# luigiba/OpenKEonSpark

Measured on AMD Instinct MI355X. Metric: positive triples/sec (training step), higher is better.
Workload: dtype f32

## Files before the change

### openkeonspark_amd/csrc/abi.hip

```cpp
#include <cstdio>
#include <cstring>
#include <iostream>

#include "engine.hpp"

namespace kge {

Engine &engine() {
    static Engine e;
    return e;
}

void set_error(const std::string &msg) {
    engine().last_error = msg;
    std::fprintf(stderr, "[kge_mi355] error: %s\n", msg.c_str());
}

int fail(int code, const std::string &msg) {
    set_error(msg);
    return code;
}

int hip_check(hipError_t e, const char *what) {
    if (e == hipSuccess) return KGE_OK;
// ... 17 lines not shown
    size_t bytes = sizeof(T) * (count ? count : 1);
    int rc = hip_check(hipMalloc(&dst, bytes), what);
    if (rc) return rc;
    if (count) rc = hip_check(hipMemcpy(dst, src, sizeof(T) * count, hipMemcpyHostToDevice), what);
    return rc;
}

int ensure_device_index() {
    Engine &e = engine();
    if (!e.index.loaded) return fail(KGE_ERR_NO_DATASET, "no training set imported (importTrainFiles / kge_import_train_arrays)");
    if (!device_ok()) return fail(KGE_ERR_NO_DEVICE, "no usable HIP device: the sampler has no CPU fallback");
    int rc = KGE_OK;
    if (!e.dev.uploaded) {
        const KgIndex &ix = e.index;
        if ((rc = upload(e.dev.pos, ix.pos.data(), ix.pos.size(), "upload pos"))) return rc;
        if ((rc = upload(e.dev.grp, ix.grp.data(), ix.grp.size(), "upload grp"))) return rc;
        if ((rc = upload(e.dev.ht, ix.ht.data(), ix.ht.size(), "upload ht"))) return rc;
        if ((rc = upload(e.dev.tails_hr, ix.tails_hr.data(), ix.tails_hr.size(), "upload tails"))) return rc;
        if ((rc = upload(e.dev.heads_tr, ix.heads_tr.data(), ix.heads_tr.size(), "upload heads"))) return rc;
        if ((rc = upload(e.dev.rels_ht, ix.rels_ht.data(), ix.rels_ht.size(), "upload rels"))) return rc;
        if ((rc = upload(e.dev.bern_prob, ix.bern_prob.data(), ix.bern_prob.size(), "upload bern"))) return rc;
        e.dev.uploaded = true;
    }
    if ((int64_t)e.streams.size() != e.work_threads) {
        e.streams.assign((size_t)e.work_threads, 0);
        e.dev.streams_sync = 0;
    }
    if (e.dev.streams_sync == 0) {
        if (e.dev.streams_cap < e.work_threads) {
            uint64_t *base = e.dev.streams < e.dev.streams_next ? e.dev.streams : e.dev.streams_next;
            if (base) (void)hipFree(base);
            e.dev.streams = e.dev.streams_next = nullptr;
            if ((rc = hip_check(hipMalloc(&e.dev.streams, sizeof(uint64_t) * 2 * (size_t)e.work_threads), "alloc streams"))) return rc;
            e.dev.streams_next = e.dev.streams + e.work_threads;
            e.dev.streams_cap = e.work_threads;
        }
        if ((rc = hip_check(hipMemcpy(e.dev.streams, e.streams.data(), sizeof(uint64_t) * (size_t)e.work_threads,
                                      hipMemcpyHostToDevice), "upload streams"))) return rc;
        e.dev.streams_sync = 1;
    }
    return KGE_OK;
}

int ensure_typed_host_index() {
    Engine &e = engine();
    if (!e.index.loaded) return fail(KGE_ERR_NO_DATASET, "type-constrained sampling: no training set imported");
// ... 31 lines not shown
    if (e.dev.streams_sync == 2) {
        int rc = hip_check(hipMemcpy(e.streams.data(), e.dev.streams, sizeof(uint64_t) * e.streams.size(),
                                     hipMemcpyDeviceToHost), "download streams");
        if (rc) return rc;
        e.dev.streams_sync = 1;
    }
    return KGE_OK;
}

static void adopt_index(KgIndex &&ix) {
    Engine &e = engine();
    e.index = std::move(ix);
    e.dev.uploaded = false;
}

static std::string build_and_adopt(int64_t E, int64_t R, int64_t nb, int64_t n, const int64_t *h, const int64_t *t, const int64_t *r) {
    Engine &e = engine();
    if (device_ok()) { (void)flush_attached_sampler(nullptr); (void)hipDeviceSynchronize(); }
    if (e.index_device_min >= 0 && n >= e.index_device_min && device_ok() && device_index_build_supported(E, R, n)) {
        KgIndex ix;
        std::string err = build_index_device(ix, e.dev, E, R, nb, n, h, t, r);
        if (!err.empty()) { e.dev.uploaded = false; return err; }
        e.index = std::move(ix);
        return "";
    }
    KgIndex ix;
    std::string err = build_index(ix, E, R, nb, n, h, t, r);
    if (!err.empty()) return err;
    adopt_index(std::move(ix));
    return "";
}

void transe_team_shape(int D, int &L, int &C);
}

using namespace kge;

extern "C" {

void setInPath(char *path) {
    engine().in_path = path ? path : "";
    std::printf("Input Files Path : %s\n", engine().in_path.c_str());
}

void setOutPath(char *path) {
    engine().out_path = path ? path : "";
    std::printf("Output Files Path : %s\n", engine().out_path.c_str());
}

void setWorkThreads(INT threads) { engine().work_threads = threads < 1 ? 1 : threads; }
INT getWorkThreads(void) { return engine().work_threads; }
void setBern(INT con) { engine().bern = con; }
// ... 55 lines not shown
    if (hip_check(hipMemcpy(batch_h, w, sizeof(int64_t) * total, hipMemcpyDeviceToHost), "copy batch_h")) return;
    if (hip_check(hipMemcpy(batch_t, w + total, sizeof(int64_t) * total, hipMemcpyDeviceToHost), "copy batch_t")) return;
    if (hip_check(hipMemcpy(batch_r, w + 2 * total, sizeof(int64_t) * total, hipMemcpyDeviceToHost), "copy batch_r")) return;
    hip_check(hipMemcpy(batch_y, w + 3 * total, sizeof(float) * total, hipMemcpyDeviceToHost), "copy batch_y");
}

size_t kge_last_error(char *buf, size_t n) {
    const std::string &s = engine().last_error;
    if (buf && n) {
        size_t k = s.size() < n - 1 ? s.size() : n - 1;
        std::memcpy(buf, s.data(), k);
        buf[k] = 0;
    }
    return s.size();
}

void kge_clear_error(void) { engine().last_error.clear(); }
int kge_device_available(void) { return device_ok() ? 1 : 0; }
const char *kge_version(void) { return "kge_mi355 0.1 (gfx950)"; }

int kge_set_option(const char *name, INT value) {
    std::string n = name ? name : "";
    if (n == "counts_force_sort") { engine().counts_force_sort = value != 0; return KGE_OK; }
    if (n == "ride_shares") { engine().ride_shares = (int)value; return KGE_OK; }
    if (n == "transr_bf16x3") { engine().transr_bf16x3 = value != 0; return KGE_OK; }
    if (n == "transr_groups") { engine().transr_groups = (int)value; return KGE_OK; }
    if (n == "transr_fuse_vec") { engine().transr_fuse_vec = value != 0; return KGE_OK; }
    if (n == "counts_fused") { engine().counts_fused = value != 0; return KGE_OK; }
    if (n == "counts_fused_diag") { engine().counts_fused_diag = (int)value; return KGE_OK; }
    if (n == "counts_fused_cap") { engine().counts_fused_cap = value > 0 ? (int)value : 0; return KGE_OK; }
    if (n == "inv_table_max_bytes") { engine().inv_table_max_bytes = value; return KGE_OK; }
    if (n == "tables_changed") { tables_written(); return KGE_OK; }
    if (n == "counts_krel") { int k = 1; while (k * 2 <= value && k < 64) k *= 2; engine().counts_krel = k; return KGE_OK; }
    if (n == "inv_carry") { engine().inv_carry = value != 0; tables_written(); return KGE_OK; }
    if (n == "emit_rounds") { engine().emit_rounds = value != 0; return KGE_OK; }
    if (n == "emit_pack") { engine().emit_pack = value != 0; return KGE_OK; }
    if (n == "float_records") { engine().float_records = value != 0; return KGE_OK; }
    if (n == "float_records_min") { engine().float_records_min = value; return KGE_OK; }
    if (n == "index_device_min") { engine().index_device_min = value; return KGE_OK; }
    if (n == "hub_copies") { engine().hub_copies = value != 0; return KGE_OK; }
    if (n == "pair_counts") { engine().pair_counts = value != 0; return KGE_OK; }
    if (n == "record_emit_event") { engine().record_emit_event = value != 0; return KGE_OK; }
    if (n == "transr_dgrad_records") { engine().transr_dgrad_records = value != 0; return KGE_OK; }
    if (n == "transr_dgrad_records_min") { engine().transr_dgrad_records_min = value; return KGE_OK; }
    if (n == "transr_lean") { engine().transr_lean = value != 0; return KGE_OK; }
    if (n == "pair_counts_min_neg") { engine().pair_counts_min_neg = (int)value; return KGE_OK; }
// ... 51 lines not shown
int kge_import_train_arrays(INT ent_total, INT rel_total, INT n, const INT *h, const INT *t, const INT *r,
                            INT new_batch_total) {
    std::string err = build_and_adopt(ent_total, rel_total, new_batch_total, n, (const int64_t *)h, (const int64_t *)t,
                                      (const int64_t *)r);
    if (!err.empty()) return fail(KGE_ERR_BAD_ARG, err);
    return KGE_OK;
}

int64_t kge_index_copy(const char *what, void *dst, int64_t bytes) {
    const KgIndex &ix = engine().index;
    if (!ix.loaded) return fail(KGE_ERR_NO_DATASET, "kge_index_copy: no dataset");
    const void *src = nullptr;
    int64_t have = 0;
    std::string w = what ? what : "";
    const bool typed = w == "type_tails" || w == "type_heads" || w == "type_bounds" || w == "typed_pos_hr" || w == "typed_pos_tr" ||
                       w == "typed_len";
    if (typed) { int rc = ensure_typed_host_index(); if (rc) return rc; }
#define KGE_ARR(name, vec) if (w == name) { src = (vec).data(); have = (int64_t)((vec).size() * sizeof((vec)[0])); }
    KGE_ARR("tails_hr", ix.tails_hr) KGE_ARR("heads_tr", ix.heads_tr) KGE_ARR("rels_ht", ix.rels_ht)
    KGE_ARR("pos", ix.pos) KGE_ARR("grp", ix.grp) KGE_ARR("ht", ix.ht)
    KGE_ARR("left_mean", ix.left_mean) KGE_ARR("right_mean", ix.right_mean) KGE_ARR("bern_prob", ix.bern_prob)
    KGE_ARR("type_tails", ix.type_tails) KGE_ARR("type_heads", ix.type_heads) KGE_ARR("type_bounds", ix.type_bounds)
    KGE_ARR("typed_pos_hr", ix.typed_pos_hr) KGE_ARR("typed_pos_tr", ix.typed_pos_tr) KGE_ARR("typed_len", ix.typed_len)
#undef KGE_ARR
    if (!src && have == 0 && !typed && w != "tails_hr" && w != "heads_tr" && w != "rels_ht" && w != "pos" && w != "grp" && w != "ht" &&
        w != "left_mean" && w != "right_mean" && w != "bern_prob")
        return fail(KGE_ERR_BAD_ARG, "kge_index_copy: unknown array " + w);
    if (dst && bytes > 0 && have > 0) std::memcpy(dst, src, (size_t)(bytes < have ? bytes : have));
    return have;
}

int kge_set_typed_sampling(INT on) {
    Engine &e = engine();
    int rc = flush_attached_sampler(nullptr);
    if (rc) return rc;
    if (on && (rc = ensure_typed_host_index())) return rc;
    e.typed_sampling = on ? 1 : 0;
    return KGE_OK;
}

int kge_typed_sampling(void) { return engine().typed_sampling; }

int kge_get_stream_states(uint64_t *dst, INT n) {
    Engine &e = engine();
    int rc = pull_streams();
    if (rc) return rc;
    for (INT i = 0; i < n && i < (INT)e.streams.size(); i++) dst[i] = e.streams[(size_t)i];
    return KGE_OK;
// ... 205 lines not shown
```

### openkeonspark_amd/csrc/engine.hpp

```cpp
#pragma once
#include <hip/hip_runtime.h>

#include <cstdint>
#include <mutex>
#include <string>
#include <vector>

#include "../../include/kge_mi355.h"
#include "kg_index.hpp"

namespace kge {

struct DeviceIndex {
    bool uploaded = false;
    int4 *pos = nullptr;
    int4 *grp = nullptr;
    int2 *ht = nullptr;
    int32_t *tails_hr = nullptr, *heads_tr = nullptr, *rels_ht = nullptr;
    float *bern_prob = nullptr;
    uint64_t *streams = nullptr;
    uint64_t *streams_next = nullptr;
    int64_t streams_cap = 0;
    int streams_sync = 0;
    int32_t *stage_i32 = nullptr;
    int64_t *stage_i64 = nullptr;
    int64_t stage_cap = 0;
    float *loss_partials = nullptr;
    unsigned *loss_ticket = nullptr;
    bool typed_uploaded = false;
    int2 *typed_len = nullptr;
    int4 *type_bounds = nullptr;
    int32_t *type_tails = nullptr, *type_heads = nullptr, *typed_pos_hr = nullptr, *typed_pos_tr = nullptr;
};

struct Engine {
    std::mutex mu;
    std::string in_path = "../data/FB15K/";
    std::string out_path = "../data/FB15K/";
    int64_t work_threads = 1;
    int64_t bern = 0;
    KgIndex index;
    LibcRand libc;
    std::vector<uint64_t> streams;
    LcgJumpTable jump = make_jump_table();
    DeviceIndex dev;
    std::string last_error;
    int device_state = 0;
    int record_emit_event = 0;
    hipEvent_t emit_done = nullptr;
    unsigned long long emit_seq = 0, emit_waited = 0;
    int time_emit = 0;
    static constexpr int kEmitRing = 512;
    hipEvent_t ev_emit0[kEmitRing] = {}, ev_emit1[kEmitRing] = {};
    long long emit_launches = 0;
    long long emit_seen = 0;
    int time_sampler = 0;
    hipEvent_t ev_samp0[kEmitRing] = {}, ev_samp1[kEmitRing] = {};
    long long samp_launches = 0, samp_seen = 0;
    float *inv_norm = nullptr;
    int64_t inv_cap = 0;
    const float *inv_for_ent = nullptr, *inv_for_rel = nullptr;
    int inv_valid = 0;
    int32_t *loss_limbs = nullptr;
    int counts_krel = 4;
    int inv_carry = 1;
    int emit_rounds = 1;
    int emit_pack = 1;
// ... 124 lines not shown
```

### openkeonspark_amd/csrc/kg_index.cpp

```cpp
#include "kg_index.hpp"

#include <algorithm>
#include <cstdio>
#include <cstdlib>
#include <cstring>
#include <numeric>

namespace kge {

namespace {

bool slurp(const std::string &path, std::vector<char> &buf) {
    FILE *f = std::fopen(path.c_str(), "rb");
    if (!f) return false;
    std::fseek(f, 0, SEEK_END);
    long n = std::ftell(f);
    std::fseek(f, 0, SEEK_SET);
    buf.resize(static_cast<size_t>(n) + 1);
    size_t got = n > 0 ? std::fread(buf.data(), 1, static_cast<size_t>(n), f) : 0;
    buf[got] = 0;
    buf.resize(got + 1);
    std::fclose(f);
    return true;
}
// ... 236 lines not shown
    f_ = (f_ + 1) % 31;
    r_ = (r_ + 1) % 31;
    return int32_t(v >> 1);
}

LcgJumpTable make_jump_table() {
    LcgJumpTable tab;
    uint64_t a = kLcgMul, c = kLcgAdd;
    for (int j = 0; j < 64; j++) {
        tab.mulA[j] = a;
        tab.addC[j] = c;
        c = a * c + c;
        a = a * a;
    }
    return tab;
}

uint64_t lcg_jump(const LcgJumpTable &tab, uint64_t state, uint64_t steps) {
    for (int j = 0; steps; j++, steps >>= 1)
        if (steps & 1) state = tab.mulA[j] * state + tab.addC[j];
    return state;
}

}
```

### openkeonspark_amd/csrc/kg_index.hpp

```cpp
#pragma once
#include <cstdint>
#include <string>
#include <vector>

namespace kge {

struct Int4 { int32_t x, y, z, w; };
struct Int2 { int32_t x, y; };

struct KgIndex {
    int64_t ent_total = 0, rel_total = 0;
    int64_t train_dup = 0;
    int64_t train_uniq = 0;
    int64_t new_batch = 0;
    std::vector<Int4> pos;
    std::vector<Int4> grp;
    std::vector<Int2> ht;
    std::vector<int32_t> tails_hr;
    std::vector<int32_t> heads_tr;
    std::vector<int32_t> rels_ht;
    std::vector<float> left_mean, right_mean, bern_prob;
    bool loaded = false;
    std::vector<int32_t> type_tails, type_heads;
    std::vector<Int4> type_bounds;
    std::vector<int32_t> typed_pos_hr, typed_pos_tr;
    std::vector<Int2> typed_len;
    bool typed_built = false;
};

std::string load_openke_dir(const std::string &dir, int64_t &ent_total, int64_t &rel_total, int64_t &new_batch,
                            std::vector<int64_t> &h, std::vector<int64_t> &t, std::vector<int64_t> &r);

bool read_all_longs(const std::string &path, std::vector<int64_t> &out);

std::string build_index(KgIndex &ix, int64_t ent_total, int64_t rel_total, int64_t new_batch, int64_t n,
                        const int64_t *h, const int64_t *t, const int64_t *r);

void relation_means(KgIndex &ix, const std::vector<int64_t> &freq_rel, const std::vector<int64_t> &groups_hr,
                    const std::vector<int64_t> &groups_tr);

std::string build_typed_index(KgIndex &ix, const std::vector<int32_t> &head_lef, const std::vector<int32_t> &head_rig,
                              const std::vector<int32_t> &head_type, const std::vector<int32_t> &tail_lef,
                              const std::vector<int32_t> &tail_rig, const std::vector<int32_t> &tail_type);

class LibcRand {
   public:
    LibcRand();
    int32_t next();

   private:
    uint32_t s_[31];
    int f_, r_;
};

constexpr uint64_t kLcgMul = 25214903917ULL;
constexpr uint64_t kLcgAdd = 11ULL;
struct LcgJumpTable { uint64_t mulA[64]; uint64_t addC[64]; };
LcgJumpTable make_jump_table();
uint64_t lcg_jump(const LcgJumpTable &tab, uint64_t state, uint64_t steps);

inline void thread_slice(int64_t batch, int64_t threads, int64_t id, int64_t &lef, int64_t &rig) {
    if (batch % threads == 0) {
        lef = id * (batch / threads);
        rig = (id + 1) * (batch / threads);
    } else {
        lef = id * (batch / threads + 1);
        rig = (id + 1) * (batch / threads + 1);
        if (rig > batch) rig = batch;
        if (lef > batch) lef = batch;
    }
}

}
```

### openkeonspark_amd/csrc/persist.hip

```cpp
#include "models_dev.hpp"
#include "optim_dev.hpp"
#include "sampler_dev.hpp"
#include "team_shape.hpp"

namespace kge {
namespace {

constexpr int kLine = 32;
constexpr unsigned kSpinLimit = 1u << 22;

struct GridBarrier {
    unsigned xcd_count[8 * kLine];
    unsigned xcd_gen[8 * kLine];
    unsigned xcd_pop[8 * kLine];
    unsigned top_count[kLine];
    unsigned flat[kLine];
    unsigned abort_flag[kLine];
};

__device__ __forceinline__ unsigned ld_agent(const unsigned *p) { return __hip_atomic_load(p, __ATOMIC_RELAXED, __HIP_MEMORY_SCOPE_AGENT); }

struct BarrierState {
    unsigned xcc, pop, n_xcd, gen;
};
// ... 330 lines not shown
                if (g_hub_auxr) (void)hipFree(g_hub_auxr);
                g_hub_rel = g_hub_auxr = nullptr;
                g_hub_elems = copies * per_copy;
                if ((rc = hip_check(hipMalloc(&g_hub_rel, sizeof(float) * (size_t)g_hub_elems), "alloc hub copies"))) return rc;
                if ((rc = hip_check(hipMalloc(&g_hub_auxr, sizeof(float) * (size_t)g_hub_elems), "alloc hub copies"))) return rc;
                if ((rc = hip_check(hipMemset(g_hub_rel, 0, sizeof(float) * (size_t)g_hub_elems), "zero hub copies"))) return rc;
                if ((rc = hip_check(hipMemset(g_hub_auxr, 0, sizeof(float) * (size_t)g_hub_elems), "zero hub copies"))) return rc;
            }
            a.copies_rel = g_hub_rel; a.copies_auxr = g_hub_auxr; a.hub_k = (int)copies;
            pa.fold_k = (int)copies; pa.fold_elems = per_copy;
        }
    }
    SamplerArgs &s = pa.sm;
    s.pos = e.dev.pos; s.grp = e.dev.grp; s.ht = e.dev.ht;
    s.tails_hr = e.dev.tails_hr; s.heads_tr = e.dev.heads_tr; s.rels_ht = e.dev.rels_ht;
    s.bern_prob = e.dev.bern_prob; s.streams = e.dev.streams; s.streams_next = nullptr; s.W = W; s.B = B;
    s.out_h = g_batch; s.out_t = g_batch + batch_len; s.out_r = g_batch + 2 * batch_len;
    s.per_thread = (B % W == 0) ? B / W : B / W + 1; s.pos_lo = 0; s.n_local = B; s.out_stride = B;
    s.train_dup = e.index.train_dup; s.new_batch = e.index.new_batch;
    s.ent_total = (int)e.index.ent_total; s.rel_total = (int)e.index.rel_total;
    s.neg = (int)negRate; s.negrel = (int)negRelRate; s.bern = e.bern ? 1 : 0;
    s.pick_div = (unsigned long long)(s.new_batch > 0 ? s.new_batch : s.train_dup);
    s.pick_magic = ~0ull / s.pick_div;
    int kshift = 0;
    while ((1 << kshift) < 1 + negRate + negRelRate) kshift++;
    s.kshift = kshift;
    for (int i = 0; i < 4; i++) { pa.tb.p[i] = pa.tb.g[i] = pa.tb.m[i] = pa.tb.v[i] = nullptr; pa.tb.n[i] = 0; }
    for (int i = 0; i < n_tables; i++) {
        int64_t rows = 0, cols = 0;
        if (kge_table_shape(m, i, &rows, &cols)) return KGE_ERR_BAD_ARG;
        pa.tb.p[i] = tables[i]; pa.tb.g[i] = grads[i]; pa.tb.n[i] = rows * cols;
        if (adam) { pa.tb.m[i] = adam_m[i]; pa.tb.v[i] = adam_v[i]; }
        uintptr_t bits = reinterpret_cast<uintptr_t>(tables[i]) | reinterpret_cast<uintptr_t>(grads[i]);
        if (adam) bits |= reinterpret_cast<uintptr_t>(adam_m[i]) | reinterpret_cast<uintptr_t>(adam_v[i]);
        if (!tables[i] || !grads[i] || (bits & 15)) return fail(KGE_ERR_BAD_ARG, "kge_train_steps_persistent: tables must be non-null and 16-byte aligned");
    }
    pa.n_tables = n_tables; pa.adam = adam; pa.n_steps = (int)n_steps;
    pa.b1 = beta1; pa.b2 = beta2; pa.eps = eps;
    pa.lr = g_lr; pa.losses = d_losses; pa.partials = g_partials; pa.bar = g_bar;
    pa.B = B; pa.W = (int)W;
    pa.touch = e.persist_touch; pa.ahead = e.persist_ahead;
    if (e.persist_trace) {
        if (!g_trace && (rc = hip_check(hipMalloc(&g_trace, sizeof(unsigned long long) * (6 * kTraceSteps + kTraceBlocks)), "alloc phase trace"))) return rc;
        if ((rc = hip_check(hipMemsetAsync(g_trace, 0, sizeof(unsigned long long) * (6 * kTraceSteps + kTraceBlocks), stream), "zero phase trace"))) return rc;
        pa.trace = g_trace;
    }
// ... 50 lines not shown
```

### openkeonspark_amd/csrc/sampler.hip

```cpp
#include "sampler_dev.hpp"

namespace kge {

__global__ __launch_bounds__(256) void sample_kernel_wide(SamplerArgs a) { sample_block_wide(a, blockIdx.x, gridDim.x); }

__global__ __launch_bounds__(256) void sample_kernel(SamplerArgs a) {
    __shared__ float bern_lds[kBernLds];
    sample_block(a, blockIdx.x, gridDim.x, bern_lds);
}

__global__ __launch_bounds__(256) void sample_kernel_wide_typed(TypedSamplerArgs a) { sample_block_wide<true>(a, blockIdx.x, gridDim.x); }

__global__ __launch_bounds__(256) void sample_kernel_typed(TypedSamplerArgs a) {
    __shared__ float bern_lds[kBernLds];
    sample_block<true>(a, blockIdx.x, gridDim.x, bern_lds);
}

__global__ __launch_bounds__(256) void sample_kernel_part(SamplerArgs a) {
    __shared__ float bern_lds[kBernLds];
    sample_block_ride(a, blockIdx.x, bern_lds);
}

__global__ void advance_streams_kernel(uint64_t *streams, long long W, long long B, long long per_thread,
                                       unsigned long long draws) {
// ... 24 lines not shown
    const int64_t W = e.work_threads;
    if (B <= 0 || neg < 0 || negrel < 0 || thread_lo < 0 || thread_hi > W || thread_lo > thread_hi)
        return fail(KGE_ERR_BAD_ARG, "kge_sampling_device: bad batch/thread range");
    if (e.index.train_dup <= 0) return fail(KGE_ERR_NO_DATASET, "sampling: empty training set");
    if ((rc = upload_jump_table())) return rc;
    int64_t lo, hi, tmp;
    if (thread_lo == thread_hi) { lo = hi = 0; }
    else { thread_slice(B, W, thread_lo, lo, tmp); thread_slice(B, W, thread_hi - 1, tmp, hi); }
    const int64_t n_local = hi - lo;
    if (n_local_out) *n_local_out = n_local;
    if (out_stride < n_local) return fail(KGE_ERR_BAD_ARG, "kge_sampling_device: out_stride smaller than the slice");
    const int64_t per_thread = (B % W == 0) ? B / W : B / W + 1;
    a = TypedSamplerArgs();
    a.pos = e.dev.pos; a.grp = e.dev.grp; a.ht = e.dev.ht;
    a.tails_hr = e.dev.tails_hr; a.heads_tr = e.dev.heads_tr; a.rels_ht = e.dev.rels_ht;
    a.bern_prob = e.dev.bern_prob; a.streams = e.dev.streams;
    a.out_h = d_h; a.out_t = d_t; a.out_r = d_r;
    a.per_thread = per_thread; a.pos_lo = lo; a.n_local = n_local; a.out_stride = out_stride;
    a.train_dup = e.index.train_dup; a.new_batch = e.index.new_batch;
    a.ent_total = (int)e.index.ent_total; a.rel_total = (int)e.index.rel_total;
    a.neg = (int)neg; a.negrel = (int)negrel; a.bern = e.bern ? 1 : 0;
    a.pick_div = (unsigned long long)(a.new_batch > 0 ? a.new_batch : a.train_dup);
    a.pick_magic = ~0ull / a.pick_div;
    const int kshift = sampler_kshift(neg, negrel);
    a.kshift = kshift;
    a.pack = emit_pack_shape(a.ent_total, a.rel_total, neg, negrel) ? d_pack : nullptr;
    a.streams_next = e.dev.streams_next; a.W = W; a.B = B;
    if (e.typed_sampling) {
        a.typed_len = e.dev.typed_len; a.type_bounds = e.dev.type_bounds;
        a.type_tails = e.dev.type_tails; a.type_heads = e.dev.type_heads;
        a.typed_pos_hr = e.dev.typed_pos_hr; a.typed_pos_tr = e.dev.typed_pos_tr;
    }
    wide = kshift > 6;
    int64_t nb = n_local > 0 ? ((n_local << kshift) + 255) / 256 : 0;
    if (nb > (1 << 20)) nb = 1 << 20;
    blocks = (unsigned)nb;
    return KGE_OK;
}

static void launch_whole(const TypedSamplerArgs &a, unsigned blocks, bool wide, hipStream_t stream) {
    Engine &e = engine();
    const int slot = (int)(e.samp_launches % Engine::kEmitRing);
    const bool timed = e.time_sampler > 0 && (e.samp_seen++ % e.time_sampler) == 0;
    if (timed) {
        if (!e.ev_samp0[slot]) { (void)hipEventCreate(&e.ev_samp0[slot]); (void)hipEventCreate(&e.ev_samp1[slot]); }
        (void)hipEventRecord(e.ev_samp0[slot], stream);
// ... 89 lines not shown
```

### openkeonspark_amd/csrc/sampler_dev.hpp

```cpp
#pragma once
#include "engine.hpp"

namespace kge {

static __constant__ LcgJumpTable c_jump;
static bool g_jump_uploaded = false;

static inline int upload_jump_table() {
    if (g_jump_uploaded) return KGE_OK;
    int rc = hip_check(hipMemcpyToSymbol(HIP_SYMBOL(c_jump), &engine().jump, sizeof(LcgJumpTable)), "upload jump table");
    if (rc == KGE_OK) g_jump_uploaded = true;
    return rc;
}

struct SamplerArgs {
    const int4 *pos;
    const int4 *grp;
    const int2 *ht;
    const int32_t *tails_hr, *heads_tr, *rels_ht;
    const float *bern_prob;
    const uint64_t *streams;
    uint64_t *streams_next;
    long long W, B;
    int32_t *out_h, *out_t, *out_r;
    int32_t *pack;
    long long per_thread;
    long long pos_lo;
    long long n_local;
    long long out_stride;
    long long train_dup, new_batch;
    unsigned long long pick_div, pick_magic;
    int ent_total, rel_total;
    int neg, negrel, bern;
    int kshift;
    unsigned ride_first, ride_total;
};

struct TypedSamplerArgs : SamplerArgs {
    const int2 *typed_len = nullptr;
    const int4 *type_bounds = nullptr;
    const int32_t *type_tails = nullptr, *type_heads = nullptr, *typed_pos_hr = nullptr, *typed_pos_tr = nullptr;
};
template <bool TYPED> struct SamplerArgsOf { using type = SamplerArgs; };
template <> struct SamplerArgsOf<true> { using type = TypedSamplerArgs; };

__device__ __forceinline__ uint64_t lcg_step(uint64_t s) { return s * kLcgMul + kLcgAdd; }

__device__ __forceinline__ uint64_t lcg_skip(uint64_t s, uint64_t n) {
    for (int j = 0; n != 0; ++j, n >>= 1)
        if (n & 1) s = c_jump.mulA[j] * s + c_jump.addC[j];
    return s;
}

__device__ __forceinline__ uint64_t mod_magic(uint64_t s, uint64_t d, uint64_t m) {
    uint64_t r = s - __umul64hi(s, m) * d;
    while (r >= d) r -= d;
    return r;
}
__device__ __forceinline__ uint32_t mod_u64_u32(uint64_t s, uint32_t d) {
    if (d == 0) return 0;
    const double rcp = 1.0 / (double)d;
    const uint32_t hi = (uint32_t)(s >> 32), lo = (uint32_t)s;
    uint32_t q1 = (uint32_t)((double)hi * rcp);
    int64_t r1 = (int64_t)hi - (int64_t)q1 * d;
    if (r1 < 0) r1 += d;
    if (r1 >= (int64_t)d) r1 -= d;
    const uint64_t x = ((uint64_t)r1 << 32) | lo;
    const double xd = (double)(uint32_t)r1 * 4294967296.0 + (double)lo;
    uint64_t q2 = (uint64_t)(xd * rcp);
    int64_t r2 = (int64_t)(x - q2 * d);
    if (r2 < 0) r2 += d;
    if (r2 < 0) r2 += d;
    if (r2 >= (int64_t)d) r2 -= d;
    if (r2 >= (int64_t)d) r2 -= d;
    return (uint32_t)r2;
}

__device__ __forceinline__ int filtered_pick(const int32_t *__restrict__ vals, int len, long long tmp) {
    int lo = 0, hi = len;
    while (lo < hi) {
        int mid = (lo + hi) >> 1;
        if ((long long)vals[mid] - mid <= tmp) lo = mid + 1; else hi = mid;
    }
    return (int)(tmp + lo);
}

__device__ __forceinline__ int filtered_pick_short(const int32_t *__restrict__ vals, int len, long long tmp) {
    if (len > 4) return filtered_pick(vals, len, tmp);
    if (len <= 0) return (int)tmp;
    int v[4];
#pragma unroll
    for (int j = 0; j < 4; j++) v[j] = vals[j < len ? j : len - 1];
    int lo = 0;
#pragma unroll
    for (int j = 0; j < 4; j++) lo += (j < len && (long long)v[j] - j <= tmp) ? 1 : 0;
    return (int)(tmp + lo);
}

template <bool SHORT>
__device__ __forceinline__ int typed_pick(const TypedSamplerArgs &a, uint64_t s, bool new_tail, int r, const int4 &gq, const int2 &tl) {
    const int32_t *__restrict__ vals = new_tail ? a.typed_pos_hr + gq.x : a.typed_pos_tr + gq.z;
    const int len = new_tail ? tl.x : tl.y;
    int v[4] = {0, 0, 0, 0};
    if (SHORT) {
        const int last = len > 0 ? len - 1 : 0;
#pragma unroll
        for (int j = 0; j < 4; j++) v[j] = vals[j < last ? j : last];
    }
    const int4 tb = a.type_bounds[r];
    const int loff = new_tail ? tb.x : tb.z, llen = new_tail ? tb.y : tb.w;
    const int c = llen - len;
    if (c <= 0) return -1;
    const long long tmp = (long long)mod_u64_u32(s, (uint32_t)c);
    int pos;
    if (SHORT && len <= 4) {
        int lo = 0;
#pragma unroll
        for (int j = 0; j < 4; j++) lo += (j < len && (long long)v[j] - j <= tmp) ? 1 : 0;
        pos = (int)(tmp + lo);
    } else
        pos = filtered_pick(vals, len, tmp);
    pos = min(pos, llen - 1);
    return (new_tail ? a.type_tails : a.type_heads)[loff + pos];
}

__device__ __forceinline__ uint64_t lcg_skip_lanes(uint64_t s, unsigned n) {
#pragma unroll
    for (int j = 0; j < 16; j++) {
        if (!__any((n >> j) != 0u)) break;
        const uint64_t t = c_jump.mulA[j] * s + c_jump.addC[j];
        s = ((n >> j) & 1u) ? t : s;
    }
    return s;
}

template <bool TYPED = false>
__device__ __forceinline__ void sample_slot(const typename SamplerArgsOf<TYPED>::type &a, long long p, long long k, unsigned long long skip_draws, int &oh, int &ot,
                                            int &orr) {
    const long long id = (long long)((unsigned)p / (unsigned)a.per_thread);
    const long long off = p - id * a.per_thread;
    const unsigned long long draws = 1ull + 2ull * a.neg + a.negrel;
    uint64_t s = lcg_skip(a.streams[id], skip_draws + (unsigned long long)off * draws);
    s = lcg_step(s);
    long long i = (long long)mod_magic(s, a.pick_div, a.pick_magic) + (a.new_batch > 0 ? a.train_dup - a.new_batch : 0);
    const int4 tr = a.pos[i];
    const int4 gq = a.grp[i];
    int2 tl = make_int2(0, 0);
    if constexpr (TYPED) tl = a.typed_len[i];
    oh = tr.x; ot = tr.y; orr = tr.z;
    if (k >= 1 && k <= a.neg) {
        s = lcg_skip(s, 2ull * (unsigned long long)(k - 1));
        s = lcg_step(s);
        const float prob = a.bern ? a.bern_prob[orr] : 500.0f;
        const bool keep_head = (float)(s % 1000ull) < prob;
        s = lcg_step(s);
        if constexpr (TYPED) {
            const int typed_id = typed_pick<false>(a, s, keep_head, orr, gq, tl);
            if (typed_id >= 0) {
                if (keep_head) ot = typed_id; else oh = typed_id;
                return;
            }
        }
        if (keep_head) {
            long long tmp = (long long)mod_u64_u32(s, (uint32_t)(a.ent_total - gq.y));
            ot = min(filtered_pick(a.tails_hr + gq.x, gq.y, tmp), a.ent_total - 1);
        } else {
            long long tmp = (long long)mod_u64_u32(s, (uint32_t)(a.ent_total - gq.w));
            oh = min(filtered_pick(a.heads_tr + gq.z, gq.w, tmp), a.ent_total - 1);
        }
    } else if (k > a.neg) {
        s = lcg_skip(s, 2ull * a.neg + (unsigned long long)(k - 1 - a.neg));
        s = lcg_step(s);
        const int2 g = a.ht[i];
        long long tmp = (long long)mod_u64_u32(s, (uint32_t)(a.rel_total - g.y));
        orr = min(filtered_pick(a.rels_ht + g.x, g.y, tmp), a.rel_total - 1);
    }
}

__device__ __forceinline__ void write_next_streams(const SamplerArgs &a, int kp, long long block, long long n_blocks) {
    for (long long id = block * 256 + threadIdx.x; id < a.W; id += n_blocks * 256) {
        long long lef = id * a.per_thread, rig = lef + a.per_thread;
        if (rig > a.B) rig = a.B;
        if (lef > a.B) lef = a.B;
        a.streams_next[id] = lcg_skip(a.streams[id], (unsigned long long)(rig - lef) * (unsigned long long)(kp + a.neg));
    }
}

template <bool TYPED = false>
__device__ __forceinline__ void sample_block_wide(const typename SamplerArgsOf<TYPED>::type &a, long long block, long long n_blocks) {
    const int kshift = a.kshift, kp = 1 + a.neg + a.negrel;
    write_next_streams(a, kp, block, n_blocks);
    for (long long g = block * 256 + threadIdx.x; (g >> kshift) < a.n_local; g += n_blocks * 256) {
        const long long b = g >> kshift;
        const long long k = g & ((1 << kshift) - 1);
        if (k >= kp) continue;
        int oh, ot, orr;
        sample_slot<TYPED>(a, a.pos_lo + b, k, 0ull, oh, ot, orr);
        const long long o = b + k * a.out_stride;
        a.out_h[o] = oh; a.out_t[o] = ot; a.out_r[o] = orr;
    }
}

constexpr int kBernLds = 2048;

template <bool TYPED = false>
__device__ __forceinline__ void sample_block(const typename SamplerArgsOf<TYPED>::type &a, long long block, long long n_blocks, float *bern_lds) {
    const int kshift = a.kshift, kp = 1 + a.neg + a.negrel, kmask = (1 << kshift) - 1;
    const unsigned long long draws = 1ull + 2ull * a.neg + a.negrel;
    write_next_streams(a, kp, block, n_blocks);
    const bool bern_in_lds = a.bern && a.rel_total <= kBernLds;
    if (bern_in_lds) {
        for (int i = threadIdx.x; i < a.rel_total; i += 256) bern_lds[i] = a.bern_prob[i];
        __syncthreads();
    }
    const int lane = threadIdx.x & 63;
    const long long total = a.n_local << kshift;
    const long long wave0 = block * 256 + (__builtin_amdgcn_readfirstlane(threadIdx.x) & ~63);
    for (long long g0 = wave0; g0 < total; g0 += n_blocks * 256) {
        const long long p0 = a.pos_lo + (g0 >> kshift);
        const long long id0 = (long long)((unsigned)p0 / (unsigned)a.per_thread);
        const long long off0 = p0 - id0 * a.per_thread;
        const uint64_t base0 = lcg_skip(a.streams[id0], (unsigned long long)off0 * draws);
        const long long g = g0 + lane;
        long long b = g >> kshift;
        const int k = (int)(g & kmask);
        const bool live = b < a.n_local && k < kp;
        if (b >= a.n_local) b = a.n_local - 1;
        const int kk = k < kp ? k : kp - 1;
        const long long p = a.pos_lo + b;
        const long long id = (long long)((unsigned)p / (unsigned)a.per_thread);
        const long long off = p - id * a.per_thread;
        const bool same = id == id0;
        uint64_t s = same ? base0 : a.streams[id];
        unsigned ahead = (unsigned)((same ? off - off0 : off) * (long long)draws);
        if (kk >= 1) ahead += kk <= a.neg ? 1u + 2u * (unsigned)(kk - 1) : 1u + 2u * (unsigned)a.neg + (unsigned)(kk - 1 - a.neg);
        s = lcg_skip_lanes(s, ahead);
        s = lcg_step(s);
        const long long pick = (long long)mod_magic(s, a.pick_div, a.pick_magic) + (a.new_batch > 0 ? a.train_dup - a.new_batch : 0);
        const long long i = __shfl((int)pick, lane & ~kmask);
        const int4 tr = a.pos[i];
        const int4 gq = a.grp[i];
        int2 tl = make_int2(0, 0);
        if constexpr (TYPED) tl = a.typed_len[i];
        int oh = tr.x, ot = tr.y, orr = tr.z;
        if (kk >= 1 && kk <= a.neg) {
            const float prob = a.bern ? (bern_in_lds ? bern_lds[orr] : a.bern_prob[orr]) : 500.0f;
            const bool keep_head = (float)(s % 1000ull) < prob;
            s = lcg_step(s);
            int typed_id = -1;
            if constexpr (TYPED) typed_id = typed_pick<true>(a, s, keep_head, orr, gq, tl);
            if (typed_id >= 0) {
                if (keep_head) ot = typed_id; else oh = typed_id;
            } else if (keep_head) {
                const long long tmp = (long long)mod_u64_u32(s, (uint32_t)(a.ent_total - gq.y));
                ot = min(filtered_pick_short(a.tails_hr + gq.x, gq.y, tmp), a.ent_total - 1);
            } else {
                const long long tmp = (long long)mod_u64_u32(s, (uint32_t)(a.ent_total - gq.w));
                oh = min(filtered_pick_short(a.heads_tr + gq.z, gq.w, tmp), a.ent_total - 1);
            }
        } else if (kk > a.neg) {
            const int2 gr = a.ht[i];
            const long long tmp = (long long)mod_u64_u32(s, (uint32_t)(a.rel_total - gr.y));
            orr = min(filtered_pick_short(a.rels_ht + gr.x, gr.y, tmp), a.rel_total - 1);
        }
        if (live) {
            const long long o = b + (long long)k * a.out_stride;
            a.out_h[o] = oh; a.out_t[o] = ot; a.out_r[o] = orr;
        }
        if (a.pack && g < total) {
            int w = 0;
            if (live && k >= 1) {
                const NegClass nc = classify_negative<KGE_TRANSE>(tr.x, tr.y, tr.z, oh, ot, orr, 0);
                const int code = !nc.same_h ? 0 : (!nc.same_t ? 1 : 2);
                const int row = !nc.same_h ? oh : (!nc.same_t ? ot : orr);
                w = row | (code << kPackRowBits) | (nc.fast ? 0 : (int)0x80000000u);
            }
            a.pack[g] = w;
        }
    }
}


__device__ __forceinline__ void sample_block_ride(const SamplerArgs &a, long long i, float *bern_lds) {
    sample_block<false>(a, (long long)a.ride_first + i, (long long)a.ride_total, bern_lds);
}

// ... 2 lines not shown
```

Measured before the change: 159.7 million.

## Use digit jump tables, precomputed modulus magics, and wide filtered search in sampler

Replaces bit-serial LCG skip-ahead with a 4-level, 9-bit digit table of precomputed affine maps read through scalar/constant address space. It also prefetches the next iteration's stream state and jump digits before the LDS fill. Per-length magic reciprocals replace 64-bit modulo in filtered picks, and the short linear filtered pick becomes a branch-unified M-ary search shared by entity and relation negatives. This cuts the serial multiply chains and divergent branches, at the cost of extra table loads and more registers.

```diff
diff --git a/openkeonspark_amd/csrc/abi.hip b/openkeonspark_amd/csrc/abi.hip
--- a/openkeonspark_amd/csrc/abi.hip
+++ b/openkeonspark_amd/csrc/abi.hip
@@ -63,6 +63,13 @@
         if ((rc = upload(e.dev.bern_prob, ix.bern_prob.data(), ix.bern_prob.size(), "upload bern"))) return rc;
         e.dev.uploaded = true;
     }
+    if (!e.dev.tables_uploaded) {
+        const KgIndex &ix = e.index;
+        if ((rc = upload(e.dev.jump_digits, e.jump_digits.data(), e.jump_digits.size(), "upload jump digits"))) return rc;
+        if ((rc = upload(e.dev.ent_magic, ix.ent_magic.data(), ix.ent_magic.size(), "upload entity moduli"))) return rc;
+        if ((rc = upload(e.dev.rel_magic, ix.rel_magic.data(), ix.rel_magic.size(), "upload relation moduli"))) return rc;
+        e.dev.tables_uploaded = true;
+    }
     if ((int64_t)e.streams.size() != e.work_threads) {
         e.streams.assign((size_t)e.work_threads, 0);
         e.dev.streams_sync = 0;
@@ -140,12 +147,14 @@
         std::string err = build_index_device(ix, e.dev, E, R, nb, n, h, t, r);
         if (!err.empty()) { e.dev.uploaded = false; return err; }
         e.index = std::move(ix);
-        return "";
-    }
-    KgIndex ix;
-    std::string err = build_index(ix, E, R, nb, n, h, t, r);
-    if (!err.empty()) return err;
-    adopt_index(std::move(ix));
+    } else {
+        KgIndex ix;
+        std::string err = build_index(ix, E, R, nb, n, h, t, r);
+        if (!err.empty()) return err;
+        adopt_index(std::move(ix));
+    }
+    build_magic_tables(e.index, e.sampler_magic_len);
+    e.dev.tables_uploaded = false;
     return "";
 }
 
@@ -247,6 +256,14 @@
 int kge_set_option(const char *name, INT value) {
     std::string n = name ? name : "";
     if (n == "counts_force_sort") { engine().counts_force_sort = value != 0; return KGE_OK; }
+    if (n == "sampler_magic_len") {
+        Engine &e = engine();
+        if (device_ok()) { (void)flush_attached_sampler(nullptr); (void)hipDeviceSynchronize(); }
+        e.sampler_magic_len = value > 0 ? value : 0;
+        if (e.index.loaded) build_magic_tables(e.index, e.sampler_magic_len);
+        e.dev.tables_uploaded = false;
+        return KGE_OK;
+    }
     if (n == "ride_shares") { engine().ride_shares = (int)value; return KGE_OK; }
     if (n == "transr_bf16x3") { engine().transr_bf16x3 = value != 0; return KGE_OK; }
     if (n == "transr_groups") { engine().transr_groups = (int)value; return KGE_OK; }
@@ -344,8 +361,9 @@
     KGE_ARR("left_mean", ix.left_mean) KGE_ARR("right_mean", ix.right_mean) KGE_ARR("bern_prob", ix.bern_prob)
     KGE_ARR("type_tails", ix.type_tails) KGE_ARR("type_heads", ix.type_heads) KGE_ARR("type_bounds", ix.type_bounds)
     KGE_ARR("typed_pos_hr", ix.typed_pos_hr) KGE_ARR("typed_pos_tr", ix.typed_pos_tr) KGE_ARR("typed_len", ix.typed_len)
+    KGE_ARR("jump_digits", engine().jump_digits) KGE_ARR("ent_magic", ix.ent_magic) KGE_ARR("rel_magic", ix.rel_magic)
 #undef KGE_ARR
-    if (!src && have == 0 && !typed && w != "tails_hr" && w != "heads_tr" && w != "rels_ht" && w != "pos" && w != "grp" && w != "ht" &&
+    if (!src && have == 0 && !typed && w != "jump_digits" && w != "ent_magic" && w != "rel_magic" && w != "tails_hr" && w != "heads_tr" && w != "rels_ht" && w != "pos" && w != "grp" && w != "ht" &&
         w != "left_mean" && w != "right_mean" && w != "bern_prob")
         return fail(KGE_ERR_BAD_ARG, "kge_index_copy: unknown array " + w);
     if (dst && bytes > 0 && have > 0) std::memcpy(dst, src, (size_t)(bytes < have ? bytes : have));
diff --git a/openkeonspark_amd/csrc/engine.hpp b/openkeonspark_amd/csrc/engine.hpp
--- a/openkeonspark_amd/csrc/engine.hpp
+++ b/openkeonspark_amd/csrc/engine.hpp
@@ -18,6 +18,9 @@
     int2 *ht = nullptr;
     int32_t *tails_hr = nullptr, *heads_tr = nullptr, *rels_ht = nullptr;
     float *bern_prob = nullptr;
+    bool tables_uploaded = false;
+    LcgAffine *jump_digits = nullptr;
+    uint64_t *ent_magic = nullptr, *rel_magic = nullptr;
     uint64_t *streams = nullptr;
     uint64_t *streams_next = nullptr;
     int64_t streams_cap = 0;
@@ -43,6 +46,8 @@
     LibcRand libc;
     std::vector<uint64_t> streams;
     LcgJumpTable jump = make_jump_table();
+    std::vector<LcgAffine> jump_digits = make_jump_digit_table(jump);
+    int64_t sampler_magic_len = 2048;
     DeviceIndex dev;
     std::string last_error;
     int device_state = 0;
diff --git a/openkeonspark_amd/csrc/kg_index.cpp b/openkeonspark_amd/csrc/kg_index.cpp
--- a/openkeonspark_amd/csrc/kg_index.cpp
+++ b/openkeonspark_amd/csrc/kg_index.cpp
@@ -282,4 +282,27 @@
     return state;
 }
 
-}
+std::vector<LcgAffine> make_jump_digit_table(const LcgJumpTable &tab) {
+    const int n = 1 << kJumpDigitBits;
+    std::vector<LcgAffine> dig((size_t)kJumpDigitLevels * n);
+    for (int k = 0; k < kJumpDigitLevels; k++) {
+        const uint64_t a = tab.mulA[k * kJumpDigitBits], c = tab.addC[k * kJumpDigitBits];
+        LcgAffine cur = {1, 0};
+        for (int d = 0; d < n; d++) {
+            dig[(size_t)k * n + d] = cur;
+            cur = {a * cur.mul, a * cur.add + c};
+        }
+    }
+    return dig;
+}
+
+void build_magic_tables(KgIndex &ix, int64_t T) {
+    auto fill = [T](std::vector<uint64_t> &m, int64_t total) {
+        m.assign((size_t)(T < 0 ? 0 : T), 0);
+        for (int64_t len = 0; len < T && len < total; len++) m[(size_t)len] = ~0ull / (uint64_t)(total - len);
+    };
+    fill(ix.ent_magic, ix.ent_total);
+    fill(ix.rel_magic, ix.rel_total);
+}
+
+}
diff --git a/openkeonspark_amd/csrc/kg_index.hpp b/openkeonspark_amd/csrc/kg_index.hpp
--- a/openkeonspark_amd/csrc/kg_index.hpp
+++ b/openkeonspark_amd/csrc/kg_index.hpp
@@ -20,6 +20,7 @@
     std::vector<int32_t> heads_tr;
     std::vector<int32_t> rels_ht;
     std::vector<float> left_mean, right_mean, bern_prob;
+    std::vector<uint64_t> ent_magic, rel_magic;
     bool loaded = false;
     std::vector<int32_t> type_tails, type_heads;
     std::vector<Int4> type_bounds;
@@ -58,6 +59,10 @@
 struct LcgJumpTable { uint64_t mulA[64]; uint64_t addC[64]; };
 LcgJumpTable make_jump_table();
 uint64_t lcg_jump(const LcgJumpTable &tab, uint64_t state, uint64_t steps);
+constexpr int kJumpDigitBits = 9, kJumpDigitLevels = 4;
+struct LcgAffine { uint64_t mul, add; };
+std::vector<LcgAffine> make_jump_digit_table(const LcgJumpTable &tab);
+void build_magic_tables(KgIndex &ix, int64_t T);
 
 inline void thread_slice(int64_t batch, int64_t threads, int64_t id, int64_t &lef, int64_t &rig) {
     if (batch % threads == 0) {
diff --git a/openkeonspark_amd/csrc/persist.hip b/openkeonspark_amd/csrc/persist.hip
--- a/openkeonspark_amd/csrc/persist.hip
+++ b/openkeonspark_amd/csrc/persist.hip
@@ -376,6 +376,7 @@
     s.neg = (int)negRate; s.negrel = (int)negRelRate; s.bern = e.bern ? 1 : 0;
     s.pick_div = (unsigned long long)(s.new_batch > 0 ? s.new_batch : s.train_dup);
     s.pick_magic = ~0ull / s.pick_div;
+    set_sampler_tables(s);
     int kshift = 0;
     while ((1 << kshift) < 1 + negRate + negRelRate) kshift++;
     s.kshift = kshift;
diff --git a/openkeonspark_amd/csrc/sampler.hip b/openkeonspark_amd/csrc/sampler.hip
--- a/openkeonspark_amd/csrc/sampler.hip
+++ b/openkeonspark_amd/csrc/sampler.hip
@@ -70,6 +70,7 @@
     a.neg = (int)neg; a.negrel = (int)negrel; a.bern = e.bern ? 1 : 0;
     a.pick_div = (unsigned long long)(a.new_batch > 0 ? a.new_batch : a.train_dup);
     a.pick_magic = ~0ull / a.pick_div;
+    set_sampler_tables(a);
     const int kshift = sampler_kshift(neg, negrel);
     a.kshift = kshift;
     a.pack = emit_pack_shape(a.ent_total, a.rel_total, neg, negrel) ? d_pack : nullptr;
diff --git a/openkeonspark_amd/csrc/sampler_dev.hpp b/openkeonspark_amd/csrc/sampler_dev.hpp
--- a/openkeonspark_amd/csrc/sampler_dev.hpp
+++ b/openkeonspark_amd/csrc/sampler_dev.hpp
@@ -34,7 +34,16 @@
     int neg, negrel, bern;
     int kshift;
     unsigned ride_first, ride_total;
+    const LcgAffine *jump_digits;
+    const uint64_t *ent_magic, *rel_magic;
+    int magic_len;
 };
+
+static inline void set_sampler_tables(SamplerArgs &a) {
+    const Engine &e = engine();
+    a.jump_digits = e.dev.jump_digits; a.ent_magic = e.dev.ent_magic; a.rel_magic = e.dev.rel_magic;
+    a.magic_len = (int)e.sampler_magic_len;
+}
 
 struct TypedSamplerArgs : SamplerArgs {
     const int2 *typed_len = nullptr;
@@ -50,6 +59,30 @@
     for (int j = 0; n != 0; ++j, n >>= 1)
         if (n & 1) s = c_jump.mulA[j] * s + c_jump.addC[j];
     return s;
+}
+
+typedef unsigned long long u64x2 __attribute__((ext_vector_type(2)));
+__device__ __forceinline__ u64x2 jump_digit(const LcgAffine *dig, int level, unsigned d) {
+    return ((const __attribute__((address_space(4))) u64x2 *)dig)[(level << kJumpDigitBits) + (int)(d & ((1u << kJumpDigitBits) - 1u))];
+}
+struct LcgJump { u64x2 e0, e1, e2, e3; };
+__device__ __forceinline__ LcgJump lcg_jump_request(const LcgAffine *dig, uint64_t n) {
+    LcgJump j;
+    j.e0 = jump_digit(dig, 0, (unsigned)n); j.e1 = jump_digit(dig, 1, (unsigned)(n >> kJumpDigitBits));
+    j.e2 = j.e3 = u64x2{1ull, 0ull};
+    if (n >> (2 * kJumpDigitBits)) {
+        j.e2 = jump_digit(dig, 2, (unsigned)(n >> (2 * kJumpDigitBits))); j.e3 = jump_digit(dig, 3, (unsigned)(n >> (3 * kJumpDigitBits)));
+    }
+    return j;
+}
+__device__ __forceinline__ uint64_t lcg_jump_apply(const LcgJump &j, uint64_t s, uint64_t n) {
+    if (n >> (kJumpDigitBits * kJumpDigitLevels)) return lcg_skip(s, n);
+    s = j.e1.x * (j.e0.x * s + j.e0.y) + j.e1.y;
+    if (n >> (2 * kJumpDigitBits)) s = j.e3.x * (j.e2.x * s + j.e2.y) + j.e3.y;
+    return s;
+}
+__device__ __forceinline__ uint64_t lcg_skip_tab(const LcgAffine *dig, uint64_t s, uint64_t n) {
+    return lcg_jump_apply(lcg_jump_request(dig, n), s, n);
 }
 
 __device__ __forceinline__ uint64_t mod_magic(uint64_t s, uint64_t d, uint64_t m) {
@@ -85,16 +118,45 @@
     return (int)(tmp + lo);
 }
 
-__device__ __forceinline__ int filtered_pick_short(const int32_t *__restrict__ vals, int len, long long tmp) {
-    if (len > 4) return filtered_pick(vals, len, tmp);
-    if (len <= 0) return (int)tmp;
-    int v[4];
-#pragma unroll
-    for (int j = 0; j < 4; j++) v[j] = vals[j < len ? j : len - 1];
-    int lo = 0;
-#pragma unroll
-    for (int j = 0; j < 4; j++) lo += (j < len && (long long)v[j] - j <= tmp) ? 1 : 0;
-    return (int)(tmp + lo);
+constexpr int kPickFan =
+#ifdef KGE_PICK_FAN
+    KGE_PICK_FAN;
+#else
+    4;
+#endif
+template <int M>
+__device__ __forceinline__ int filtered_pick_wide(const int32_t *__restrict__ vals, int len, int total, const uint64_t *__restrict__ magic,
+                                                  int magic_len, uint64_t s) {
+    int lo = 0, hi = len, v[M];
+    int step = (len + M) / (M + 1);
+    const int last = len > 0 ? len - 1 : 0;
+#pragma unroll
+    for (int j = 0; j < M; j++) v[j] = vals[min((j + 1) * step - 1 < 0 ? 0 : (j + 1) * step - 1, last)];
+    const uint32_t d = (uint32_t)(total - len);
+    int tmp;
+    if (len < magic_len) {
+        const uint64_t m = magic[len];
+        uint64_t r = s - __umul64hi(s, m) * d;
+        if (r >= d) r -= d;
+        if (r >= d) r -= d;
+        tmp = d == 0 ? 0 : (int)r;
+    } else
+        tmp = (int)mod_u64_u32(s, d);
+    while (lo < hi) {
+        int t = 0;
+#pragma unroll
+        for (int j = 0; j < M; j++) {
+            const int p = lo + (j + 1) * step - 1;
+            t += (p < hi && v[j] - p <= tmp) ? 1 : 0;
+        }
+        lo += t * step;
+        if (t < M) hi = min(hi, lo + step - 1);
+        if (lo >= hi) break;
+        step = (hi - lo + M) / (M + 1);
+#pragma unroll
+        for (int j = 0; j < M; j++) v[j] = vals[min(lo + (j + 1) * step - 1, hi - 1)];
+    }
+    return tmp + lo;
 }
 
 template <bool SHORT>
@@ -124,23 +186,13 @@
     return (new_tail ? a.type_tails : a.type_heads)[loff + pos];
 }
 
-__device__ __forceinline__ uint64_t lcg_skip_lanes(uint64_t s, unsigned n) {
-#pragma unroll
-    for (int j = 0; j < 16; j++) {
-        if (!__any((n >> j) != 0u)) break;
-        const uint64_t t = c_jump.mulA[j] * s + c_jump.addC[j];
-        s = ((n >> j) & 1u) ? t : s;
-    }
-    return s;
-}
-
 template <bool TYPED = false>
 __device__ __forceinline__ void sample_slot(const typename SamplerArgsOf<TYPED>::type &a, long long p, long long k, unsigned long long skip_draws, int &oh, int &ot,
                                             int &orr) {
     const long long id = (long long)((unsigned)p / (unsigned)a.per_thread);
     const long long off = p - id * a.per_thread;
     const unsigned long long draws = 1ull + 2ull * a.neg + a.negrel;
-    uint64_t s = lcg_skip(a.streams[id], skip_draws + (unsigned long long)off * draws);
+    uint64_t s = lcg_skip_tab(a.jump_digits, a.streams[id], skip_draws + (unsigned long long)off * draws);
     s = lcg_step(s);
     long long i = (long long)mod_magic(s, a.pick_div, a.pick_magic) + (a.new_batch > 0 ? a.train_dup - a.new_batch : 0);
     const int4 tr = a.pos[i];
@@ -149,7 +201,7 @@
     if constexpr (TYPED) tl = a.typed_len[i];
     oh = tr.x; ot = tr.y; orr = tr.z;
     if (k >= 1 && k <= a.neg) {
-        s = lcg_skip(s, 2ull * (unsigned long long)(k - 1));
+        s = lcg_skip_tab(a.jump_digits, s, 2ull * (unsigned long long)(k - 1));
         s = lcg_step(s);
         const float prob = a.bern ? a.bern_prob[orr] : 500.0f;
         const bool keep_head = (float)(s % 1000ull) < prob;
@@ -169,7 +221,7 @@
             oh = min(filtered_pick(a.heads_tr + gq.z, gq.w, tmp), a.ent_total - 1);
         }
     } else if (k > a.neg) {
-        s = lcg_skip(s, 2ull * a.neg + (unsigned long long)(k - 1 - a.neg));
+        s = lcg_skip_tab(a.jump_digits, s, 2ull * a.neg + (unsigned long long)(k - 1 - a.neg));
         s = lcg_step(s);
         const int2 g = a.ht[i];
         long long tmp = (long long)mod_u64_u32(s, (uint32_t)(a.rel_total - g.y));
@@ -208,60 +260,87 @@
     const int kshift = a.kshift, kp = 1 + a.neg + a.negrel, kmask = (1 << kshift) - 1;
     const unsigned long long draws = 1ull + 2ull * a.neg + a.negrel;
     write_next_streams(a, kp, block, n_blocks);
+    const int lane = threadIdx.x & 63;
+    const long long total = a.n_local << kshift;
+    const long long wave0 = block * 256 + (__builtin_amdgcn_readfirstlane(threadIdx.x) & ~63);
+    struct Slots {
+        unsigned long long n0;
+        uint64_t st0, st;
+        LcgJump jump0;
+        u64x2 j0, j1;
+        long long b;
+        int k, kk;
+        bool live, same;
+    };
+    auto request = [&](long long g0) {
+        Slots w;
+        const long long p0 = a.pos_lo + (g0 >> kshift);
+        const long long id0 = (long long)((unsigned)p0 / (unsigned)a.per_thread);
+        const long long off0 = p0 - id0 * a.per_thread;
+        w.n0 = (unsigned long long)off0 * draws;
+        w.jump0 = lcg_jump_request(a.jump_digits, w.n0);
+        w.st0 = ((const __attribute__((address_space(4))) uint64_t *)a.streams)[id0];
+        const long long g = g0 + lane;
+        w.b = g >> kshift;
+        w.k = (int)(g & kmask);
+        w.live = w.b < a.n_local && w.k < kp;
+        if (w.b >= a.n_local) w.b = a.n_local - 1;
+        w.kk = w.k < kp ? w.k : kp - 1;
+        const long long p = a.pos_lo + w.b;
+        const long long id = (long long)((unsigned)p / (unsigned)a.per_thread);
+        const long long off = p - id * a.per_thread;
+        w.same = id == id0;
+        unsigned ahead = (unsigned)((w.same ? off - off0 : off) * (long long)draws);
+        if (w.kk >= 1) ahead += w.kk <= a.neg ? 1u + 2u * (unsigned)(w.kk - 1) : 1u + 2u * (unsigned)a.neg + (unsigned)(w.kk - 1 - a.neg);
+        w.j0 = jump_digit(a.jump_digits, 0, ahead); w.j1 = jump_digit(a.jump_digits, 1, ahead >> kJumpDigitBits);
+        w.st = 0;
+        if (!w.same) w.st = a.streams[id];
+        return w;
+    };
+    Slots w = request(wave0 < total ? wave0 : 0);
     const bool bern_in_lds = a.bern && a.rel_total <= kBernLds;
     if (bern_in_lds) {
         for (int i = threadIdx.x; i < a.rel_total; i += 256) bern_lds[i] = a.bern_prob[i];
         __syncthreads();
     }
-    const int lane = threadIdx.x & 63;
-    const long long total = a.n_local << kshift;
-    const long long wave0 = block * 256 + (__builtin_amdgcn_readfirstlane(threadIdx.x) & ~63);
     for (long long g0 = wave0; g0 < total; g0 += n_blocks * 256) {
-        const long long p0 = a.pos_lo + (g0 >> kshift);
-        const long long id0 = (long long)((unsigned)p0 / (unsigned)a.per_thread);
-        const long long off0 = p0 - id0 * a.per_thread;
-        const uint64_t base0 = lcg_skip(a.streams[id0], (unsigned long long)off0 * draws);
-        const long long g = g0 + lane;
-        long long b = g >> kshift;
-        const int k = (int)(g & kmask);
-        const bool live = b < a.n_local && k < kp;
-        if (b >= a.n_local) b = a.n_local - 1;
-        const int kk = k < kp ? k : kp - 1;
-        const long long p = a.pos_lo + b;
-        const long long id = (long long)((unsigned)p / (unsigned)a.per_thread);
-        const long long off = p - id * a.per_thread;
-        const bool same = id == id0;
-        uint64_t s = same ? base0 : a.streams[id];
-        unsigned ahead = (unsigned)((same ? off - off0 : off) * (long long)draws);
-        if (kk >= 1) ahead += kk <= a.neg ? 1u + 2u * (unsigned)(kk - 1) : 1u + 2u * (unsigned)a.neg + (unsigned)(kk - 1 - a.neg);
-        s = lcg_skip_lanes(s, ahead);
+        if (g0 != wave0) w = request(g0);
+        const long long g = g0 + lane, b = w.b;
+        const int k = w.k, kk = w.kk;
+        const bool live = w.live;
+        uint64_t s = w.same ? lcg_jump_apply(w.jump0, w.st0, w.n0) : w.st;
+        s = w.j1.x * (w.j0.x * s + w.j0.y) + w.j1.y;
         s = lcg_step(s);
         const long long pick = (long long)mod_magic(s, a.pick_div, a.pick_magic) + (a.new_batch > 0 ? a.train_dup - a.new_batch : 0);
         const long long i = __shfl((int)pick, lane & ~kmask);
         const int4 tr = a.pos[i];
-        const int4 gq = a.grp[i];
+        int4 gq = a.grp[i];
+        int2 gr = make_int2(0, 0);
+        if (a.negrel > 0) gr = a.ht[i];
+        asm volatile("" : "+v"(gq.x), "+v"(gq.y), "+v"(gq.z), "+v"(gq.w), "+v"(gr.x), "+v"(gr.y));
         int2 tl = make_int2(0, 0);
         if constexpr (TYPED) tl = a.typed_len[i];
         int oh = tr.x, ot = tr.y, orr = tr.z;
-        if (kk >= 1 && kk <= a.neg) {
-            const float prob = a.bern ? (bern_in_lds ? bern_lds[orr] : a.bern_prob[orr]) : 500.0f;
-            const bool keep_head = (float)(s % 1000ull) < prob;
-            s = lcg_step(s);
+        if (kk >= 1) {
+            const bool ent = kk <= a.neg;
+            bool keep_head = false;
             int typed_id = -1;
-            if constexpr (TYPED) typed_id = typed_pick<true>(a, s, keep_head, orr, gq, tl);
-            if (typed_id >= 0) {
-                if (keep_head) ot = typed_id; else oh = typed_id;
-            } else if (keep_head) {
-                const long long tmp = (long long)mod_u64_u32(s, (uint32_t)(a.ent_total - gq.y));
-                ot = min(filtered_pick_short(a.tails_hr + gq.x, gq.y, tmp), a.ent_total - 1);
-            } else {
-                const long long tmp = (long long)mod_u64_u32(s, (uint32_t)(a.ent_total - gq.w));
-                oh = min(filtered_pick_short(a.heads_tr + gq.z, gq.w, tmp), a.ent_total - 1);
+            if (ent) {
+                const float prob = a.bern ? (bern_in_lds ? bern_lds[orr] : a.bern_prob[orr]) : 500.0f;
+                keep_head = (float)(s % 1000ull) < prob;
+                s = lcg_step(s);
+                if constexpr (TYPED) typed_id = typed_pick<true>(a, s, keep_head, orr, gq, tl);
             }
-        } else if (kk > a.neg) {
-            const int2 gr = a.ht[i];
-            const long long tmp = (long long)mod_u64_u32(s, (uint32_t)(a.rel_total - gr.y));
-            orr = min(filtered_pick_short(a.rels_ht + gr.x, gr.y, tmp), a.rel_total - 1);
+            int v = typed_id;
+            if (typed_id < 0) {
+                const int32_t *vals = !ent ? a.rels_ht + gr.x : (keep_head ? a.tails_hr + gq.x : a.heads_tr + gq.z);
+                const int len = !ent ? gr.y : (keep_head ? gq.y : gq.w);
+                const int total = ent ? a.ent_total : a.rel_total;
+                v = min(filtered_pick_wide<kPickFan>(vals, len, total, ent ? a.ent_magic : a.rel_magic, a.magic_len, s), total - 1);
+            }
+            orr = ent ? orr : v;
+            ot = ent && keep_head ? v : ot;
+            oh = ent && !keep_head ? v : oh;
         }
         if (live) {
             const long long o = b + (long long)k * a.out_stride;
```

New measurement: 166.1 million (median of 6 runs). 4.0% higher.
